# danaesavi/SocialMedia-TextImage-Classification-AuxLosses

Measured on AMD Instinct MI355X. Metric: posts/sec (fwd+bwd) Bernice+ViT-B/16 attn-fusion, bs=64, higher is better.
Workload: dtype bf16; 1 GPU; BASELINE config 2: Bernice+ViT-B/16, attention fusion, no aux loss, bs=64/GPU; step=full train step: fwd + loss + bwd + grad exchange + AdamW + weight refresh, posts_per_gpu=64, image=224, vocab=250002, parallelism=dp1, weights=random-init at true shapes

## Files before the change

socialmedia-textimage-classification-auxlosses_amd/csrc/engine.hip:

```cpp
#include <string>
#include <vector>
#include <cstdlib>
#include <cstdio>
#include "mmhip_common.h"
#include "mmhip_host.h"

using namespace mmhip;

namespace {

struct LayerOff {
    size_t qkv_w, qkv_b, ao_w, ao_b, ln1_w, ln1_b, fc1_w, fc1_b, fc2_w, fc2_b, ln2_w, ln2_b, begin, end;
};
struct LayerW16 {
    size_t qkv, ao, fc1, fc2, qkvT, aoT, fc1T, fc2T;
};
struct TextAct {
    size_t qkv, ctx, pre1, a1, u, h, pre2, out, mean1, rstd1, mean2, rstd2, lse;
    size_t a1p, outp;
};

}

struct mmhip_engine {
// ... 12 lines not shown
    size_t x3_ws[3] = {0, 0, 0}, x3_bytes[3] = {0, 0, 0};
    size_t patch_w16;
    std::vector<TextAct> tact;
    size_t ids_all, mask_all, pos_ids, maskbias, x0, xhat_emb, rstd_emb, x0p = 0;
    bool px = false;
    int bwd_np = 3;
    size_t v_patches, v_pe, v_x, v_ln, v_qkv, v_ctx, v_h, v_out;
    size_t g_partial, g_partial_side, g_det_rows = 0;
    size_t g_lnp[2][2];
    uint8_t* word_row_state = nullptr;
    unsigned* bad_index = nullptr;
    unsigned* guard = nullptr;
    size_t g_set[2][6];
    size_t g_dx, g_dx2, g_dpre, g_ddrop, g_dpre1, g_ddrop1, g_dqkv, g_dctx, g_du;
    size_t h_vpool, h_tpool, h_txt_e, h_img_e, h_txt_n, h_img_n, h_txt_inv, h_img_inv, h_logits;
    size_t h_q, h_qk, h_prob, h_xbar, h_z, h_feats, h_featd, h_out_cls, h_out_tim;
    size_t splitk_ws = 0, splitk_ws_vit = 0; bool has_splitk = false;
    size_t h_d_out_cls, h_d_logits, h_d_out_tim, h_dfeats, h_dpre, h_dz, h_dxcls, h_dxbar, h_dqk, h_dq, h_dtxt_e, h_dimg_e,
        h_dtpool, h_dprepool, h_loss;
    int B = 0, T = 0, Bt = 0; bool itm = false, train_mode = false, fwd_done = false, bwd_begun = false;
    bool skip_itc = false, itc_done = false;
    uint64_t seed = 0;
    size_t ws_base = 0;
    int itc_max_world = 0, itc_world = 1, itc_rank = 0;
    size_t h_g_txt = 0, h_g_img = 0, h_g_rowlse = 0, h_g_collse = 0, h_g_loss = 0, h_g_dtn = 0, h_g_din = 0, h_g_ws = 0;
    bool bd_itc_global = false; float bd_w_itc = 0.f;
    const float *bd_out_cls = nullptr, *bd_logits = nullptr, *bd_out_tim = nullptr, *bd_feats = nullptr;
    hipStream_t side = nullptr;
    int vision_ready_B = 0;
    bool vit_is_long = false;
    hipStream_t side_vit[2] = {nullptr, nullptr};
    hipEvent_t ev_fork = nullptr, ev_vit = nullptr, ev_ready[2] = {nullptr, nullptr}, ev_tn[2] = {nullptr, nullptr};
    hipEvent_t ev_layer[2] = {nullptr, nullptr}, ev_opt = nullptr;
    bool tn_pending[2] = {false, false};
    int cls_only = -1;
    bool cls_compact = false;
    int overlap = -1;
    int part[2] = {-1, -1}, cur_part[2] = {0, 0}; bool part_auto = false;
    int part_bwd = -1;
    int spans_on = 0; hipEvent_t span_ev[6] = {nullptr, nullptr, nullptr, nullptr, nullptr, nullptr}; bool span_set[6] = {false, false, false, false, false, false};
    int span(int i, hipStream_t s) {
        if (!spans_on) return 0;
        if (!span_ev[i]) { hipError_t r = hipEventCreate(&span_ev[i]); if (r != hipSuccess) return (int)r; }
        hipError_t r = hipEventRecord(span_ev[i], s);
        span_set[i] = r == hipSuccess;
        return (int)r;
    }
    int timing = 0;
    struct Ev { hipEvent_t a, b; double flops; int M, N, K, flags, tile, cus; };
    std::vector<Ev> evs; size_t ev_used = 0;

    template <typename U> U* wsp(size_t off) const { return reinterpret_cast<U*>(ws + off); }
    int dt() const { return cfg.dtype; }
    bool clip() const { return cfg.img_kind == MMHIP_IMG_CLIP; }
    int Hv() const { return cfg.hidden_img > 0 ? cfg.hidden_img : cfg.hidden; }
    int Iv() const { return cfg.inter_img > 0 ? cfg.inter_img : cfg.inter; }
    int heads_v() const { return cfg.heads_img > 0 ? cfg.heads_img : cfg.heads; }
    int P() const { return (cfg.image / cfg.patch) * (cfg.image / cfg.patch) + 1; }
    int Kp() const { return 3 * cfg.patch * cfg.patch; }
    int Kpp() const { return (Kp() + 63) / 64 * 64; }
    size_t v_pre_ln_w = 0, v_pre_ln_b = 0;
    float gscale() const { return cfg.loss_scale > 0.f ? cfg.loss_scale : (cfg.dtype == MMHIP_F16 ? 1024.f : 1.f); }
    size_t esz() const { return cfg.dtype == MMHIP_BF16X3 ? 4 : 2; }
};

namespace {

void add_text_layer(ParamTable& b, const mmhip_config& c, int l, LayerOff& o) {
    const int H = c.hidden, I = c.inter;
    const std::string p = "dual_encoder.text_model.encoder.layer." + std::to_string(l) + ".";
    const int g = MMHIP_G_ALWAYS;
    o.begin = b.off[1];
    o.qkv_w = b.add(p + "attention.self.query.weight", 1, g, {H, H});
// ... 245 lines not shown
int run_gemm_pair(mmhip_engine& e, G& g0, G& g1, hipStream_t s) {
    const bool pairable = (e.dt() == DT_BF16 || e.dt() == DT_F16 || (e.dt() == DT_F32 && g0.a.a_pair && g1.a.a_pair)) && g0.a.N == g1.a.N && g0.a.K == g1.a.K;
    mmhip_engine::Ev* ev = nullptr;
    if (e.timing && pairable) {
        if (e.ev_used == e.evs.size()) {
            mmhip_engine::Ev n;
            CHECK_HIP(hipEventCreate(&n.a));
            CHECK_HIP(hipEventCreate(&n.b));
            e.evs.push_back(n);
        }
        ev = &e.evs[e.ev_used];
        CHECK_HIP(hipEventRecord(ev->a, s));
    }
    if (pairable && launch_gemm_nt8_pair(g0.a, g1.a, e.dt(), 0, s)) {
        CHECK_HIP(hipGetLastError());
        if (ev) {
            ev->flops = 2.0 * ((double)g0.a.M + g1.a.M) * (double)g0.a.N * g0.a.K;
            ev->M = g0.a.M + g1.a.M; ev->N = g0.a.N; ev->K = g0.a.K; ev->flags = g0.a.flags | g1.a.flags; ev->tile = -2; ev->cus = 0;
            CHECK_HIP(hipEventRecord(ev->b, s));
            e.ev_used++;
        }
        return 0;
    }
    CHECK_RC(run_gemm(e, g0, s));
    return run_gemm(e, g1, s);
}

int side_init(mmhip_engine& e) {
    if (e.overlap < 0) { const char* v = getenv("MMHIP_OVERLAP"); e.overlap = v ? atoi(v) : 1; }
    if (!e.overlap || e.side) return 0;
    CHECK_HIP(pool_stream(POOL_SIDE, &e.side));
    CHECK_HIP(pool_stream(POOL_VIT, &e.side_vit[0]));
    CHECK_HIP(pool_stream(POOL_VIT_HI, &e.side_vit[1]));
    hipEvent_t* evs[9] = {&e.ev_fork, &e.ev_vit, &e.ev_ready[0], &e.ev_ready[1], &e.ev_tn[0], &e.ev_tn[1], &e.ev_layer[0], &e.ev_layer[1], &e.ev_opt};
    for (auto ev : evs) CHECK_HIP(hipEventCreateWithFlags(ev, hipEventDisableTiming));
    return 0;
}
inline bool use_side(const mmhip_engine& e) { return e.overlap > 0 && e.side && e.timing != 2; }

int refresh_layer(mmhip_engine& e, const float* base, const LayerOff& o, const LayerW16& w, bool transposed, hipStream_t s, int H, int I) {
    CastMat m[4] = {{base + o.qkv_w, e.ws + w.qkv, transposed ? e.ws + w.qkvT : nullptr, 3 * H, H, 0},
                    {base + o.ao_w, e.ws + w.ao, transposed ? e.ws + w.aoT : nullptr, H, H, 0},
                    {base + o.fc1_w, e.ws + w.fc1, transposed ? e.ws + w.fc1T : nullptr, I, H, 0},
                    {base + o.fc2_w, e.ws + w.fc2, transposed ? e.ws + w.fc2T : nullptr, H, I, 0}};
    CHECK_HIP(launch_cast_group(m, 4, e.px ? DT_PAIR : e.dt(), s));
    return 0;
}

int vit_forward(mmhip_engine& e, const float* pixels, hipStream_t s) {
    const mmhip_config& c = e.cfg;
    const int H = e.Hv(), I = e.Iv(), B = e.B, P = e.P(), Kpp = e.Kpp(), dt = e.dt();
    const int Mv = B * P;
    const bool clip = e.clip();
    const float* F = e.frozen;
    const bool px = e.px;
    CHECK_HIP(launch_patchify(pixels, e.ws + e.v_patches, B, c.image, c.patch, Kpp, px ? DT_PAIR : dt, s));
    {
        G g(e.ws + e.v_patches, Kpp, e.ws + e.patch_w16, Kpp, e.ws + e.v_pe, H, B * (P - 1), H, Kpp);
        if (!clip) g.bias(F + e.v_patch_b);
        g.px_in(px);
        part_gemm(e, g, 1);
        CHECK_RC(run_gemm(e, g, s));
    }
    CHECK_HIP(launch_vit_assemble(e.ws + e.v_pe, F + e.v_cls, F + e.v_pos, e.ws + e.v_x, B, P, H, dt, s));
    char* x = e.ws + e.v_x;
    if (clip) {
        LNArgs ln{x, x, F + e.v_pre_ln_w, F + e.v_pre_ln_b, nullptr, nullptr, Mv, H, H, H, c.ln_eps_img};
// ... 259 lines not shown
        CHECK_HIP(launch_fusion_attn_fwd(fa, dt, s));
        CHECK_HIP(launch_small_nt(small(e.wsp<float>(e.h_xbar), H, W + e.fv_w, H, W + e.fv_b, z + H, ZW, Bt, H, H), DT_F32, s));
    } else {
        CHECK_HIP(launch_gather_rows_f32(e.ws + e.v_out, (size_t)P * Hv, z + H, ZW, B, Hv, dt, s));
        if (Bt > B) CHECK_HIP(launch_gather_rows_f32(e.ws + e.v_out, (size_t)P * Hv, z + (size_t)B * ZW + H, ZW, B, Hv, dt, s));
    }
    float* feats = e.wsp<float>(e.h_feats);
    CHECK_HIP(launch_small_nt(small(z, ZW, W + e.fus_w, ZW, W + e.fus_b, feats, H, Bt, H, ZW, ACT_RELU), DT_F32, s));
    CHECK_HIP(launch_elementwise(EW_DROPOUT, feats, nullptr, e.wsp<float>(e.h_featd), (size_t)B * H, 0.f,
                                 make_drop(c.p_head, e.seed, STREAM_HEAD, e.train_mode), s));
    CHECK_HIP(launch_small_nt(small(e.wsp<float>(e.h_featd), H, W + e.cls_w, H, W + e.cls_b, e.wsp<float>(e.h_out_cls), C, B, C, H), DT_F32, s));
    if (e.itm) CHECK_HIP(launch_small_nt(small(feats + (size_t)B * H, H, W + e.tim_w, H, W + e.tim_b, e.wsp<float>(e.h_out_tim), 2, B, 2, H), DT_F32, s));
    if (out_cls) CHECK_HIP(hipMemcpyAsync(out_cls, e.ws + e.h_out_cls, (size_t)B * C * 4, hipMemcpyDeviceToDevice, s));
    if (logits && e.itc_done) CHECK_HIP(hipMemcpyAsync(logits, e.ws + e.h_logits, (size_t)B * B * 4, hipMemcpyDeviceToDevice, s));
    if (out_tim && e.itm) CHECK_HIP(hipMemcpyAsync(out_tim, e.ws + e.h_out_tim, (size_t)B * 2 * 4, hipMemcpyDeviceToDevice, s));
    if (feats_out) CHECK_HIP(hipMemcpyAsync(feats_out, feats, (size_t)B * H * 4, hipMemcpyDeviceToDevice, s));
    return 0;
}

int heads_backward(mmhip_engine& e, hipStream_t s) {
    const mmhip_config& c = e.cfg;
    const int H = c.hidden, E = c.proj_dim, C = c.num_labels, T = e.T, B = e.B, Bt = e.Bt, dt = e.dt();
    const int P = e.P(), Hv = e.Hv(), ZW = H + Hv;
    const float* W = e.train;
    float* Gd = e.grad;
    const float* d_out_cls = e.bd_out_cls ? e.bd_out_cls : e.wsp<float>(e.h_d_out_cls);
    const float* d_logits = e.bd_logits;
    const float* d_out_tim = e.bd_out_tim;
    float* dfeats = e.wsp<float>(e.h_dfeats);
    float* feats = e.wsp<float>(e.h_feats);
    float* z = e.wsp<float>(e.h_z);
    float* dxcls = e.wsp<float>(e.h_dxcls);
    const DropCfg nodrop = make_drop(0.f, 0, 0, false);
    CHECK_HIP(launch_small_nn(small(d_out_cls, C, W + e.cls_w, H, nullptr, dfeats, H, B, H, C), s));
    CHECK_HIP(launch_elementwise(EW_DROPOUT, dfeats, nullptr, dfeats, (size_t)B * H, 0.f, make_drop(c.p_head, e.seed, STREAM_HEAD, e.train_mode), s));
    if (e.bd_feats) CHECK_HIP(launch_elementwise(EW_ADD, dfeats, e.bd_feats, dfeats, (size_t)B * H, 1.f, nodrop, s));
    CHECK_HIP(launch_small_tn(small(d_out_cls, C, e.wsp<float>(e.h_featd), H, nullptr, Gd + e.cls_w, H, B, H, 0, 0, 1), DT_F32, C, s));
    CHECK_HIP(launch_bias_grad_f32(d_out_cls, B, C, C, Gd + e.cls_b, 1, s));
    if (e.itm) {
        if (d_out_tim) {
            CHECK_HIP(launch_small_nn(small(d_out_tim, 2, W + e.tim_w, H, nullptr, dfeats + (size_t)B * H, H, B, H, 2), s));
            CHECK_HIP(launch_small_tn(small(d_out_tim, 2, feats + (size_t)B * H, H, nullptr, Gd + e.tim_w, H, B, H, 0, 0, 1), DT_F32, 2, s));
            CHECK_HIP(launch_bias_grad_f32(d_out_tim, B, 2, 2, Gd + e.tim_b, 1, s));
        } else {
            CHECK_HIP(hipMemsetAsync(dfeats + (size_t)B * H, 0, (size_t)B * H * 4, s));
        }
    }
    float* dpre = e.wsp<float>(e.h_dpre);
    CHECK_HIP(launch_elementwise(EW_RELU_BWD, dfeats, feats, dpre, (size_t)Bt * H, 0.f, nodrop, s));
    CHECK_HIP(launch_small_tn(small(dpre, H, z, ZW, nullptr, Gd + e.fus_w, ZW, Bt, ZW, 0, 0, 1), DT_F32, H, s));
    CHECK_HIP(launch_bias_grad_f32(dpre, Bt, H, H, Gd + e.fus_b, 1, s));
    float* dz = e.wsp<float>(e.h_dz);
    CHECK_HIP(launch_small_nn(small(dpre, H, W + e.fus_w, ZW, nullptr, dz, ZW, Bt, ZW, H), s));
    CHECK_HIP(hipMemcpy2DAsync(dxcls, (size_t)H * 4, dz, (size_t)ZW * 4, (size_t)H * 4, Bt, hipMemcpyDeviceToDevice, s));
    if (c.fusion == MMHIP_FUSION_ATTENTION) {
        const float* dctx = dz + H;
        float* q = e.wsp<float>(e.h_q);
        CHECK_HIP(launch_small_tn(small(dctx, ZW, e.wsp<float>(e.h_xbar), H, nullptr, Gd + e.fv_w, H, Bt, H, 0, 0, 1), DT_F32, H, s));
        CHECK_HIP(launch_bias_grad_f32(dctx, Bt, H, ZW, Gd + e.fv_b, 1, s));
        CHECK_HIP(launch_small_nn(small(dctx, ZW, W + e.fv_w, H, nullptr, e.wsp<float>(e.h_dxbar), H, Bt, H, H), s));
        FusionAttnBwdArgs fb{e.wsp<float>(e.h_dxbar), e.wsp<float>(e.h_prob), e.ws + e.v_out, e.wsp<float>(e.h_dqk), Bt, B, P, H, 1.0f / sqrtf((float)H)};
        CHECK_HIP(launch_fusion_attn_bwd(fb, dt, s));
        CHECK_HIP(launch_small_tn(small(q, H, e.wsp<float>(e.h_dqk), H, nullptr, Gd + e.fk_w, H, Bt, H, 0, 0, 1), DT_F32, H, s));
        CHECK_HIP(launch_small_nt(small(e.wsp<float>(e.h_dqk), H, W + e.fk_w, H, nullptr, e.wsp<float>(e.h_dq), H, Bt, H, H), DT_F32, s));
        CHECK_HIP(launch_small_tn(small(e.wsp<float>(e.h_dq), H, z, ZW, nullptr, Gd + e.fq_w, H, Bt, H, 0, 0, 1), DT_F32, H, s));
        CHECK_HIP(launch_bias_grad_f32(e.wsp<float>(e.h_dq), Bt, H, H, Gd + e.fq_b, 1, s));
        CHECK_HIP(launch_small_nn(small(e.wsp<float>(e.h_dq), H, W + e.fq_w, H, nullptr, dxcls, H, Bt, H, H, ACT_NONE, 1), s));
    }
    if (d_logits || e.bd_itc_global) {
        if (e.bd_itc_global) {
            const int G = e.itc_world * B;
            ItcGlobalBwdArgs gb{};
            gb.txt_n = e.wsp<float>(e.h_g_txt); gb.img_n = e.wsp<float>(e.h_g_img); gb.logit_scale = W + e.logit_scale;
            gb.rowlse = e.wsp<float>(e.h_g_rowlse); gb.collse = e.wsp<float>(e.h_g_collse);
            gb.txt_inv = e.wsp<float>(e.h_txt_inv); gb.img_inv = e.wsp<float>(e.h_img_inv);
            gb.d_txt_n = e.wsp<float>(e.h_g_dtn); gb.d_img_n = e.wsp<float>(e.h_g_din);
            gb.dtxt_e = e.wsp<float>(e.h_dtxt_e); gb.dimg_e = e.wsp<float>(e.h_dimg_e); gb.dlogit_scale = Gd + e.logit_scale;
            gb.ws = e.wsp<float>(e.h_g_ws); gb.G = G; gb.E = E; gb.Bl = B; gb.r0 = e.itc_rank * B;
            gb.scale = e.bd_w_itc * (float)e.itc_world / (2.f * (float)G);
            CHECK_HIP(launch_itc_global_bwd(gb, s));
        } else {
            ItcBwdArgs ib{d_logits, e.wsp<float>(e.h_logits), e.wsp<float>(e.h_txt_n), e.wsp<float>(e.h_img_n), e.wsp<float>(e.h_txt_inv),
                          e.wsp<float>(e.h_img_inv), W + e.logit_scale, e.wsp<float>(e.h_dtxt_e), e.wsp<float>(e.h_dimg_e), Gd + e.logit_scale, B, E};
            CHECK_HIP(launch_itc_bwd(ib, s));
        }
        CHECK_HIP(launch_small_tn(small(e.wsp<float>(e.h_dtxt_e), E, e.wsp<float>(e.h_tpool), H, nullptr, Gd + e.tproj_w, H, B, H, 0, 0, 1), DT_F32, E, s));
        CHECK_HIP(launch_small_tn(small(e.wsp<float>(e.h_dimg_e), E, e.wsp<float>(e.h_vpool), Hv, nullptr, Gd + e.vproj_w, Hv, B, Hv, 0, 0, 1), DT_F32, E, s));
        CHECK_HIP(launch_small_nn(small(e.wsp<float>(e.h_dtxt_e), E, W + e.tproj_w, H, nullptr, e.wsp<float>(e.h_dtpool), H, B, H, E), s));
        CHECK_HIP(launch_elementwise(EW_TANH_BWD, e.wsp<float>(e.h_dtpool), e.wsp<float>(e.h_tpool), e.wsp<float>(e.h_dprepool), (size_t)B * H, 0.f, nodrop, s));
        CHECK_HIP(launch_small_tn(small(e.wsp<float>(e.h_dprepool), H, z, ZW, nullptr, Gd + e.t_pool_w, H, B, H, 0, 0, 1), DT_F32, H, s));
        CHECK_HIP(launch_bias_grad_f32(e.wsp<float>(e.h_dprepool), B, H, H, Gd + e.t_pool_b, 1, s));
        CHECK_HIP(launch_small_nn(small(e.wsp<float>(e.h_dprepool), H, W + e.t_pool_w, H, nullptr, dxcls, H, B, H, H, ACT_NONE, 1), s));
    }
    CHECK_HIP(launch_scatter_cls_rows(dxcls, e.ws + e.g_dx, Bt, e.cls_compact ? 1 : T, H, dt, s, e.gscale()));
    return 0;
}

int text_layer_backward(mmhip_engine& e, int l, hipStream_t s) {
    const mmhip_config& c = e.cfg;
    const int H = c.hidden, I = c.inter, T = e.T, Bt = e.Bt, Mt = Bt * T, dt = e.dt();
    const float* W = e.train;
    float* Gd = e.grad;
    const LayerOff& o = e.txt[l];
    const LayerW16& w = e.txt_w16[l];
    const TextAct& a = e.tact[l];
    const bool px = e.px;
    const int np = e.bwd_np;
    const bool hi1 = px && np == 1;
    const char* x_in = px ? (l ? e.ws + e.tact[l - 1].outp : e.ws + e.x0p) : (l ? e.ws + e.tact[l - 1].out : e.ws + e.x0);
    const bool tr = e.train_mode;
    const int set = l & 1;
    const bool side = use_side(e);
    const bool compact = e.cls_compact && l == c.layers_txt - 1;
    const int Mr = compact ? Bt : Mt, rs = compact ? T * H : H, rmul = compact ? T : 1;
    char *dx = e.ws + e.g_dx, *dx2 = e.ws + e.g_dx2, *dctx = e.ws + e.g_dctx;
    char *dpre2 = e.ws + e.g_set[set][0], *ddrop2 = e.ws + e.g_set[set][1], *du = e.ws + e.g_set[set][2];
    char *dpre1 = e.ws + e.g_set[set][3], *ddrop1 = e.ws + e.g_set[set][4], *dqkv = e.ws + e.g_set[set][5];
    if (side && e.tn_pending[set]) {
        CHECK_HIP(hipStreamWaitEvent(s, e.ev_tn[set], 0));
        e.tn_pending[set] = false;
    }
    const DropCfg d_ffn = make_drop(c.p_hidden, e.seed, stream_ffn_out(l), tr);
    LNBwdArgs b2{dx, e.ws + a.pre2, W + o.ln2_w, e.wsp<float>(a.mean2), e.wsp<float>(a.rstd2), dpre2, nullptr, Gd + o.ln2_w, Gd + o.ln2_b, Mr, H,
                 e.wsp<float>(e.g_lnp[set][0]), 1.0f / e.gscale(), d_ffn.thresh16 ? ddrop2 : nullptr, nullptr, d_ffn, rmul, 1};
    ln_bwd_pair(b2, px, ddrop2, hi1);
    CHECK_HIP(launch_layernorm_bwd(b2, dt, s));
    const char* df = (px || d_ffn.thresh16) ? ddrop2 : dpre2;
    if (e.part_bwd < 0) { const char* v = getenv("MMHIP_PART_BWD"); e.part_bwd = v ? atoi(v) : 0; }
    static int bwd_mask = -1;
    if (bwd_mask < 0) { const char* v = getenv("MMHIP_PART_BWD_MASK"); bwd_mask = v ? atoi(v) : 15; }
    auto part_bwd = [&](G& g, int bit) {
        if (e.part_bwd > 0 && (bwd_mask & bit) && side && g.a.M >= 2048 && g.a.N % 256 == 0 && g.a.K % 64 == 0 && (dt == DT_BF16 || dt == DT_F16)) g.tile(15).grid(e.part_bwd);
    };
    { G g(df, H, e.ws + w.fc2T, H, du, I, Mr, I, H); g.mul_gelu_grad(e.ws + a.u, I).px_in(px, np).px_out(px, hi1); part_bwd(g, 1); CHECK_RC(run_gemm(e, g, s)); }
    static int bt12 = -1;
    if (bt12 < 0) { const char* v = getenv("MMHIP_BWD_TILE12"); bt12 = v ? atoi(v) : 1; }
    const int nt = (bt12 && Mr >= 4096 && Mr <= 8192 && H % 96 == 0) ? 12 : 0;
    { G g(du, I, e.ws + w.fc1T, I, dx2, H, Mr, H, I); g.residual(dpre2, H).px_in(px, np); g.tile(nt); part_bwd(g, 2); CHECK_RC(run_gemm(e, g, s)); }
    const DropCfg d_ao = make_drop(c.p_hidden, e.seed, stream_attn_out(l), tr);
    LNBwdArgs b1{dx2, e.ws + a.pre1, W + o.ln1_w, e.wsp<float>(a.mean1), e.wsp<float>(a.rstd1), dpre1, nullptr, Gd + o.ln1_w, Gd + o.ln1_b, Mr, H,
                 e.wsp<float>(e.g_lnp[set][1]), 1.0f / e.gscale(), d_ao.thresh16 ? ddrop1 : nullptr, nullptr, d_ao, rmul, 1};
    ln_bwd_pair(b1, px, ddrop1, hi1);
    CHECK_HIP(launch_layernorm_bwd(b1, dt, s));
    const char* dout = (px || d_ao.thresh16) ? ddrop1 : dpre1;
    if (compact) {
        { G g(dout, H, e.ws + w.aoT, H, dx2, H, Mr, H, H); g.px_in(px, np).px_out(px, hi1); CHECK_RC(run_gemm(e, g, s)); }
        CHECK_HIP(hipMemsetAsync(dctx, 0, (size_t)Mt * H * e.esz(), s));
        CHECK_HIP(launch_scatter_rows16(dx2, dctx, Bt, (size_t)T * H, H, 0, dt, s));
        CHECK_HIP(hipMemsetAsync(dqkv, 0, (size_t)Mt * 3 * H * e.esz(), s));
    } else {
        G g(dout, H, e.ws + w.aoT, H, dctx, H, Mt, H, H);
        g.px_in(px, np).px_out(px, hi1);
        g.tile((bt12 & 2) ? nt : 0);
        part_bwd(g, 4);
        CHECK_RC(run_gemm(e, g, s));
    }
    AttnBwdArgs ab = attn_bwd_args(e.ws + a.qkv, e.wsp<float>(e.maskbias), e.ws + a.ctx, dctx, e.wsp<float>(a.lse), dqkv, Bt, T, c.heads, H,
                                   make_drop(c.p_attn, e.seed, stream_attn(l), tr));
    attn_pair(ab, px, np);
    ab.q_tiles = compact ? 1 : 0;
    CHECK_HIP(launch_attn_bwd(ab, dt, s));
    hipStream_t ps = s;
    if (side) {
        CHECK_HIP(hipEventRecord(e.ev_ready[set], s));
        CHECK_HIP(hipStreamWaitEvent(e.side, e.ev_ready[set], 0));
        ps = e.side;
    }
    if (compact) {
        { G g(dqkv, 3 * H, e.ws + w.qkvT, 3 * H, dx, H, Mt, H, 3 * H); g.px_in(px, np); CHECK_RC(run_gemm(e, g, s)); }
        CHECK_HIP(launch_scatter_rows16(dpre1, dx, Bt, (size_t)T * H, H, 1, dt, s));
    } else {
        G g(dqkv, 3 * H, e.ws + w.qkvT, 3 * H, dx, H, Mt, H, 3 * H);
        g.residual(dpre1, H).px_in(px, np);
        g.tile(nt);
        part_bwd(g, 8);
        CHECK_RC(run_gemm(e, g, s));
    }
    GemmTNProblem pr[4];
    CHECK_HIP(launch_layernorm_bwd_reduce(b2, ps));
    CHECK_HIP(launch_layernorm_bwd_reduce(b1, ps));
    pr[0] = GemmTNProblem{df, e.ws + a.h, Gd + o.fc2_w, Mr, H, I, H, I, I, 0, Gd + o.fc2_b};
    pr[1] = GemmTNProblem{du, e.ws + a.a1, Gd + o.fc1_w, Mr, I, H, I, H, H, 0, Gd + o.fc1_b};
    pr[2] = GemmTNProblem{dqkv, x_in, Gd + o.qkv_w, Mt, 3 * H, H, 3 * H, H, H, 0, Gd + o.qkv_b};
    pr[3] = GemmTNProblem{dout, e.ws + a.ctx, Gd + o.ao_w, Mr, H, H, H, rs, H, 0, Gd + o.ao_b};
    if (px) {
        pr[1].B = e.ws + a.a1p;
        for (auto& q : pr) tn_pair(q, np);
    }
    {
        const int i = e.side && ps == e.side ? 1 : 0;
        CHECK_HIP(launch_gemm_tn(pr, 4, 0, dt, 0, ps, 1.0f / e.gscale(), e.x3_bytes[i] ? e.ws + e.x3_ws[i] : nullptr, e.x3_bytes[i]));
    }
    if (side) {
        CHECK_HIP(hipEventRecord(e.ev_tn[set], e.side));
        e.tn_pending[set] = true;
    }
    return 0;
}

int backward_finish(mmhip_engine& e, hipStream_t s) {
    for (int set = 0; set < 2; ++set)
        if (e.tn_pending[set]) {
            CHECK_HIP(hipStreamWaitEvent(s, e.ev_tn[set], 0));
            e.tn_pending[set] = false;
        }
    return 0;
}

static unsigned* g_nonfinite = nullptr;
static unsigned* g_skip = nullptr;
inline unsigned* guard_counter(const mmhip_engine& e) { return e.guard ? e.guard : g_nonfinite; }
inline unsigned* guard_flag(const mmhip_engine& e) { return e.guard ? e.guard + 1 : g_skip; }

int embed_backward(mmhip_engine& e, hipStream_t s) {
    const mmhip_config& c = e.cfg;
    const float* W = e.train;
    float* Gd = e.grad;
    EmbedBwdArgs b{};
    b.dx = e.ws + e.g_dx; b.xhat = e.ws + e.xhat_emb; b.rstd = e.wsp<float>(e.rstd_emb); b.gamma = W + e.t_eln_w;
    b.ids = e.wsp<int64_t>(e.ids_all); b.pos_ids = e.wsp<int>(e.pos_ids);
    b.dword = Gd + e.t_word; b.dpos = Gd + e.t_pos; b.dtype = Gd + e.t_type; b.dgamma = Gd + e.t_eln_w; b.dbeta = Gd + e.t_eln_b;
    b.posts = e.Bt; b.T = e.T; b.H = c.hidden; b.pad_id = c.pad_id;
    b.pos_pad_id = c.txt_kind == MMHIP_TXT_XLMR ? c.pad_id : -1;
    b.drop = make_drop(c.p_hidden, e.seed, STREAM_EMBED, e.train_mode);
    b.partial = e.wsp<float>(e.g_partial);
    b.alpha = 1.0f / e.gscale();
    b.row_state = e.word_row_state;
    if (deterministic()) { b.det_rows = e.wsp<float>(e.g_det_rows); b.max_pos = c.max_pos; }
    b.status = guard_flag(e) ? guard_counter(e) : nullptr;
    CHECK_HIP(launch_embed_bwd(b, e.dt(), s));
    return 0;
}

// ... 4 lines not shown
const char* mmhip_version(void) { return "mmhip 0.1 (gfx950)"; }

int mmhip_create(const mmhip_config* cfg, mmhip_handle* out) {
    if (!cfg || !out) return MMHIP_E_INVALID;
    const mmhip_config& c = *cfg;
    if (c.hidden <= 0 || c.hidden % 64 || c.hidden > 1024 || c.heads * 64 != c.hidden || c.inter % 128 || c.hidden % 128) return MMHIP_E_INVALID;
    {
        const int hv = c.hidden_img > 0 ? c.hidden_img : c.hidden, iv = c.inter_img > 0 ? c.inter_img : c.inter, nh = c.heads_img > 0 ? c.heads_img : c.heads;
        if (c.img_kind != MMHIP_IMG_VIT && c.img_kind != MMHIP_IMG_CLIP) return MMHIP_E_INVALID;
        if (hv % 128 || hv > 1024 || nh * 64 != hv || iv % 128 || c.patch < 2 || c.image % c.patch) return MMHIP_E_INVALID;
        if (c.fusion == MMHIP_FUSION_ATTENTION && hv != c.hidden) return MMHIP_E_INVALID;
        const int P = (c.image / c.patch) * (c.image / c.patch) + 1;
        if (P > 608) return MMHIP_E_INVALID;
    }
    if (c.max_text_len > 128 || c.max_text_len < 1 || c.max_posts < 1 || c.max_posts > 1024) return MMHIP_E_INVALID;
    if (c.dtype != MMHIP_BF16 && c.dtype != MMHIP_F16 && c.dtype != MMHIP_BF16X3) return MMHIP_E_INVALID;
    if (c.num_labels < 1 || c.num_labels > 64 || c.proj_dim < 1 || c.proj_dim > 1024) return MMHIP_E_INVALID;
    if (c.txt_kind == MMHIP_TXT_XLMR && c.max_pos < c.max_text_len + c.pad_id + 1) return MMHIP_E_INVALID;
    if (c.txt_kind == MMHIP_TXT_BERT && c.max_pos < c.max_text_len) return MMHIP_E_INVALID;
    mmhip_engine* e = new (std::nothrow) mmhip_engine();
    if (!e) return MMHIP_E_INVALID;
    e->cfg = c;
    if (c.dtype == MMHIP_BF16X3) { const char* v = getenv("MMHIP_X3_PAIRS"); e->px = v ? atoi(v) != 0 : true; }
    if (c.dtype == MMHIP_BF16X3) { const char* v = getenv("MMHIP_X3_BWD"); const int n = v ? atoi(v) : 3; e->bwd_np = n >= 1 && n <= 3 ? n : 3; }
    build_layout(*e);
    build_workspace(*e);
    *out = e;
    return 0;
}
void mmhip_destroy(mmhip_handle h) {
    if (!h) return;
    if (h->side) {
        (void)hipStreamSynchronize(h->side);
        for (hipEvent_t ev : {h->ev_fork, h->ev_vit, h->ev_ready[0], h->ev_ready[1], h->ev_tn[0], h->ev_tn[1], h->ev_layer[0], h->ev_layer[1], h->ev_opt})
            if (ev) (void)hipEventDestroy(ev);
        for (auto sv : h->side_vit) if (sv) (void)hipStreamSynchronize(sv);
        for (auto ev : h->span_ev) if (ev) (void)hipEventDestroy(ev);
    }
    for (auto& ev : h->evs) { (void)hipEventDestroy(ev.a); (void)hipEventDestroy(ev.b); }
    delete h;
}
int mmhip_param_count(mmhip_handle h) { return h ? (int)h->params.size() : MMHIP_E_INVALID; }
int mmhip_param_info_at(mmhip_handle h, int i, mmhip_param_info* out) {
    if (!h || !out || i < 0 || i >= (int)h->params.size()) return MMHIP_E_INVALID;
    *out = h->params[i];
    return 0;
}
uint64_t mmhip_buffer_numel(mmhip_handle h, int buffer) { return !h ? 0 : (buffer == 0 ? h->n_frozen : h->n_train); }
uint64_t mmhip_workspace_bytes(mmhip_handle h) { return h ? h->ws_need : 0; }
int mmhip_reserve_itc_global(mmhip_handle h, int max_world) {
    if (!h || max_world < 0) return MMHIP_E_INVALID;
    if (h->ws) return MMHIP_E_STATE;
    mmhip_engine& e = *h;
    const size_t Bm = e.cfg.max_posts, E = e.cfg.proj_dim, Gm = (size_t)max_world * Bm;
    if (max_world > 1 && Gm > (size_t)ITC_GLOBAL_MAX_G) return MMHIP_E_INVALID;
    e.itc_max_world = max_world > 1 ? max_world : 0;
    e.itc_world = 1; e.itc_rank = 0;
    e.ws_need = e.ws_base;
    if (!e.itc_max_world) return 0;
    Carver w;
    w.off = e.ws_base;
    e.h_g_txt = w.take(Gm * E * 4); e.h_g_img = w.take(Gm * E * 4); e.h_g_rowlse = w.take(Gm * 4); e.h_g_collse = w.take(Gm * 4); e.h_g_loss = w.take(16);
    e.h_g_dtn = w.take(Bm * E * 4); e.h_g_din = w.take(Bm * E * 4); e.h_g_ws = w.take(itc_global_ws_floats((int)Gm, (int)Bm) * 4);
    e.ws_need = w.off;
    return 0;
}
int mmhip_set_itc_global(mmhip_handle h, int world, int rank) {
// ... 173 lines not shown
    a.n_correct = n_correct;
    a.B = e.B; a.C = e.cfg.num_labels;
    CHECK_HIP(launch_loss(a, s));
    if (loss) CHECK_HIP(hipMemcpyAsync(loss, a.loss, 16, hipMemcpyDeviceToDevice, s));
    e.bd_out_cls = a.d_out_cls; e.bd_logits = a.d_logits; e.bd_out_tim = a.d_out_tim; e.bd_feats = nullptr;
    e.bd_itc_global = glob; e.bd_w_itc = w_itc;
    return 0;
}

int mmhip_num_backward_stages(mmhip_handle h) { return h ? h->cfg.layers_txt + 2 : MMHIP_E_INVALID; }

int mmhip_stage_grad_range(mmhip_handle h, int stage, uint64_t* begin, uint64_t* end) {
    if (!h || !begin || !end || stage < 0 || stage > h->cfg.layers_txt + 1) return MMHIP_E_INVALID;
    const mmhip_engine& e = *h;
    if (stage == 0) { *begin = e.heads_begin; *end = e.heads_end; }
    else if (stage <= e.cfg.layers_txt) { const LayerOff& o = e.txt[e.cfg.layers_txt - stage]; *begin = o.begin; *end = o.end; }
    else { *begin = e.emb_begin; *end = e.emb_end; }
    return 0;
}

int mmhip_backward_begin(mmhip_handle h, const float* d_out_cls, const float* d_logits, const float* d_out_tim, const float* d_feats, void* stream) {
    if (!h || !h->fwd_done || !h->grad) return MMHIP_E_STATE;
    mmhip_engine& e = *h;
    if (unsigned* f = guard_flag(e)) CHECK_HIP(hipMemsetAsync(f, 0, 4, (hipStream_t)stream));
    if (d_out_cls || d_logits || d_out_tim || d_feats) {
        if (!d_out_cls) return MMHIP_E_INVALID;
        e.bd_out_cls = d_out_cls; e.bd_logits = d_logits; e.bd_out_tim = d_out_tim; e.bd_feats = d_feats;
        e.bd_itc_global = false;
    } else if (!e.bd_out_cls) {
        return MMHIP_E_STATE;
    }
    e.bwd_begun = true;
    e.tn_pending[0] = e.tn_pending[1] = false;
    return side_init(e);
}
int mmhip_backward_stage(mmhip_handle h, int stage, void* stream) {
    if (!h || !h->bwd_begun) return MMHIP_E_STATE;
    mmhip_engine& e = *h;
    hipStream_t s = (hipStream_t)stream;
    const int L = e.cfg.layers_txt;
    if (stage == 0) return heads_backward(e, s);
    if (stage >= 1 && stage <= L) return text_layer_backward(e, L - stage, s);
    if (stage == L + 1) return embed_backward(e, s);
    return MMHIP_E_INVALID;
}
int mmhip_backward_join_stage(mmhip_handle h, int stage, void* stream) {
    if (!h || !h->bwd_begun) return MMHIP_E_STATE;
    mmhip_engine& e = *h;
    const int L = e.cfg.layers_txt;
    if (stage < 1 || stage > L) return 0;
    const int set = (L - stage) & 1;
    if (e.tn_pending[set]) {
        CHECK_HIP(hipStreamWaitEvent((hipStream_t)stream, e.ev_tn[set], 0));
        e.tn_pending[set] = false;
    }
    return 0;
}
int mmhip_backward_finish(mmhip_handle h, void* stream) {
    if (!h || !h->bwd_begun) return MMHIP_E_STATE;
    return backward_finish(*h, (hipStream_t)stream);
}
int mmhip_backward(mmhip_handle h, const float* d_out_cls, const float* d_logits, const float* d_out_tim, const float* d_feats, void* stream) {
    CHECK_RC(mmhip_backward_begin(h, d_out_cls, d_logits, d_out_tim, d_feats, stream));
    const int n = mmhip_num_backward_stages(h);
    for (int st = 0; st < n; ++st)
        CHECK_RC(mmhip_backward_stage(h, st, stream));
    return mmhip_backward_finish(h, stream);
}

int mmhip_set_nonfinite_counter(uint32_t* device_counter) {
    if ((uintptr_t)device_counter & 3) return MMHIP_E_INVALID;
    g_nonfinite = device_counter;
    g_skip = nullptr;
    return 0;
}
int mmhip_set_step_guard(uint32_t* device_words2) {
    if ((uintptr_t)device_words2 & 3) return MMHIP_E_INVALID;
    g_nonfinite = device_words2;
    g_skip = device_words2 ? device_words2 + 1 : nullptr;
    return 0;
}
int mmhip_set_guard(mmhip_handle h, uint32_t* device_words2) {
// ... 188 lines not shown
    for (int l = 0; l < L; ++l)
        if (!layer_done[l]) CHECK_RC(refresh_layer(e, e.train, e.txt[l], e.txt_w16[l], true, s, e.cfg.hidden, e.cfg.inter));
    if (rows_due) {
        if (cb) CHECK_RC(cb(user, MMHIP_CB_FINISH_ROWS));
        if (!e.word_row_state) return MMHIP_E_STATE;
        CHECK_RC(adamw_rows_impl(e.train + w0, e.grad + w0, adam_m + w0, adam_v + w0, (int)V, (int)H, e.word_row_state, lr, beta1, beta2, eps,
                                    weight_decay, step, grad_scale, 1, stream, gc, gf));
    }
    return e.span(5, s);
}

int mmhip_train_step(mmhip_handle h, const int64_t* ids, const int64_t* mask, const float* pixels, const int64_t* tim_ids,
                     const int64_t* tim_mask, const int64_t* lbl_tim, const int64_t* onehot, const float* class_w, int B, int T,
                     uint64_t seed, int use_itc, int use_itm, float w_cls, float w_itc, float w_itm, float* adam_m, float* adam_v,
                     float lr, float beta1, float beta2, float eps, float weight_decay, int step, float grad_scale, float* loss,
                     int* n_correct, void* stream) {
    return train_step_impl(h, ids, mask, pixels, tim_ids, tim_mask, lbl_tim, onehot, class_w, B, T, seed, use_itc, use_itm, w_cls, w_itc, w_itm,
                           adam_m, adam_v, lr, beta1, beta2, eps, weight_decay, step, grad_scale, loss, n_correct, stream, nullptr, nullptr);
}
int mmhip_train_step_dp(mmhip_handle h, const int64_t* ids, const int64_t* mask, const float* pixels, const int64_t* tim_ids,
                        const int64_t* tim_mask, const int64_t* lbl_tim, const int64_t* onehot, const float* class_w, int B, int T,
                        uint64_t seed, int use_itc, int use_itm, float w_cls, float w_itc, float w_itm, float* adam_m, float* adam_v,
                        float lr, float beta1, float beta2, float eps, float weight_decay, int step, float grad_scale, float* loss,
                        int* n_correct, void* stream, mmhip_exchange_cb on_stage, void* user) {
    if (!on_stage) return MMHIP_E_INVALID;
    return train_step_impl(h, ids, mask, pixels, tim_ids, tim_mask, lbl_tim, onehot, class_w, B, T, seed, use_itc, use_itm, w_cls, w_itc, w_itm,
                           adam_m, adam_v, lr, beta1, beta2, eps, weight_decay, step, grad_scale, loss, n_correct, stream, on_stage, user);
}

int mmhip_step_spans(mmhip_handle h, int enable, float* ms) {
    if (!h) return MMHIP_E_INVALID;
    mmhip_engine& e = *h;
    if (ms) {
        for (int i = 0; i < 5; ++i) ms[i] = -1.f;
        if (e.span_set[0]) {
            for (int i = 1; i < 6; ++i) {
                if (!e.span_set[i]) continue;
                CHECK_HIP(hipEventSynchronize(e.span_ev[i]));
                float t = 0.f;
                if (hipEventElapsedTime(&t, e.span_ev[0], e.span_ev[i]) == hipSuccess) ms[i - 1] = t;
            }
        }
    }
    e.spans_on = enable;
    if (!enable) for (int i = 0; i < 6; ++i) e.span_set[i] = false;
    return 0;
}
int mmhip_gemm_timing(mmhip_handle h, int enable, int reset, double* ms, uint64_t* launches, double* flops) {
    if (!h) return MMHIP_E_INVALID;
    mmhip_engine& e = *h;
    if (ms || launches || flops) {
        double tms = 0, tf = 0;
        for (size_t i = 0; i < e.ev_used; ++i) {
            CHECK_HIP(hipEventSynchronize(e.evs[i].b));
            float t = 0;
            CHECK_HIP(hipEventElapsedTime(&t, e.evs[i].a, e.evs[i].b));
            tms += t; tf += e.evs[i].flops;
        }
        if (ms) *ms = tms;
        if (launches) *launches = e.ev_used;
        if (flops) *flops = tf;
    }
    if (reset) e.ev_used = 0;
    e.timing = enable < 0 ? 0 : (enable > 2 ? 2 : enable);
    return 0;
}

int mmhip_gemm_timing_by_shape(mmhip_handle h, char* out, uint64_t capacity) {
    if (!h || !out || capacity < 2) return MMHIP_E_INVALID;
    mmhip_engine& e = *h;
    struct Row { int M, N, K, flags, tile, cus; int n; double ms, flops; };
    std::vector<Row> rows;
    for (size_t i = 0; i < e.ev_used; ++i) {
        const auto& ev = e.evs[i];
        CHECK_HIP(hipEventSynchronize(ev.b));
        float t = 0;
        CHECK_HIP(hipEventElapsedTime(&t, ev.a, ev.b));
        Row* r = nullptr;
// ... 22 lines not shown
```

Baseline: 6355 posts/s.

## Offload head weight-gradient GEMMs to side stream and trim CLS-only text backward

Moves the weight and bias gradient reductions of the classifier, fusion, attention-fusion and pooler heads onto the side stream, gated by an event, so they run concurrently with the data-gradient chain on the main stream. A join is added before stage 1 and in backward_finish. Separately, in the compact (CLS-only) last text layer, a lean path for non-f32 dtypes writes the attention-output backward GEMM straight into dctx and zeroes dqkv with a 2D memset, replacing the scatter path, and flags attention backward with Sq_live=1. More profiling span events are also added, at the cost of extra stream and event bookkeeping.

```diff
diff --git a/socialmedia-textimage-classification-auxlosses_amd/csrc/engine.hip b/socialmedia-textimage-classification-auxlosses_amd/csrc/engine.hip
--- a/socialmedia-textimage-classification-auxlosses_amd/csrc/engine.hip
+++ b/socialmedia-textimage-classification-auxlosses_amd/csrc/engine.hip
@@ -68,13 +68,15 @@
     hipStream_t side_vit[2] = {nullptr, nullptr};
     hipEvent_t ev_fork = nullptr, ev_vit = nullptr, ev_ready[2] = {nullptr, nullptr}, ev_tn[2] = {nullptr, nullptr};
     hipEvent_t ev_layer[2] = {nullptr, nullptr}, ev_opt = nullptr;
-    bool tn_pending[2] = {false, false};
+    hipEvent_t ev_heads_in = nullptr, ev_heads = nullptr;
+    bool tn_pending[2] = {false, false}, heads_pending = false;
     int cls_only = -1;
     bool cls_compact = false;
     int overlap = -1;
     int part[2] = {-1, -1}, cur_part[2] = {0, 0}; bool part_auto = false;
     int part_bwd = -1;
-    int spans_on = 0; hipEvent_t span_ev[6] = {nullptr, nullptr, nullptr, nullptr, nullptr, nullptr}; bool span_set[6] = {false, false, false, false, false, false};
+    static constexpr int N_SPAN = 8;
+    int spans_on = 0; hipEvent_t span_ev[N_SPAN] = {}; bool span_set[N_SPAN] = {};
     int span(int i, hipStream_t s) {
         if (!spans_on) return 0;
         if (!span_ev[i]) { hipError_t r = hipEventCreate(&span_ev[i]); if (r != hipSuccess) return (int)r; }
@@ -386,7 +388,8 @@
     CHECK_HIP(pool_stream(POOL_SIDE, &e.side));
     CHECK_HIP(pool_stream(POOL_VIT, &e.side_vit[0]));
     CHECK_HIP(pool_stream(POOL_VIT_HI, &e.side_vit[1]));
-    hipEvent_t* evs[9] = {&e.ev_fork, &e.ev_vit, &e.ev_ready[0], &e.ev_ready[1], &e.ev_tn[0], &e.ev_tn[1], &e.ev_layer[0], &e.ev_layer[1], &e.ev_opt};
+    hipEvent_t* evs[11] = {&e.ev_fork, &e.ev_vit, &e.ev_ready[0], &e.ev_ready[1], &e.ev_tn[0], &e.ev_tn[1], &e.ev_layer[0], &e.ev_layer[1], &e.ev_opt,
+                           &e.ev_heads_in, &e.ev_heads};
     for (auto ev : evs) CHECK_HIP(hipEventCreateWithFlags(ev, hipEventDisableTiming));
     return 0;
 }
@@ -712,40 +715,50 @@
     float* z = e.wsp<float>(e.h_z);
     float* dxcls = e.wsp<float>(e.h_dxcls);
     const DropCfg nodrop = make_drop(0.f, 0, 0, false);
+    const bool off = use_side(e);
+    hipStream_t ps = off ? e.side : s;
+    auto inputs_ready = [&]() -> int {
+        if (off) {
+            CHECK_HIP(hipEventRecord(e.ev_heads_in, s));
+            CHECK_HIP(hipStreamWaitEvent(e.side, e.ev_heads_in, 0));
+        }
+        return 0;
+    };
     CHECK_HIP(launch_small_nn(small(d_out_cls, C, W + e.cls_w, H, nullptr, dfeats, H, B, H, C), s));
     CHECK_HIP(launch_elementwise(EW_DROPOUT, dfeats, nullptr, dfeats, (size_t)B * H, 0.f, make_drop(c.p_head, e.seed, STREAM_HEAD, e.train_mode), s));
     if (e.bd_feats) CHECK_HIP(launch_elementwise(EW_ADD, dfeats, e.bd_feats, dfeats, (size_t)B * H, 1.f, nodrop, s));
-    CHECK_HIP(launch_small_tn(small(d_out_cls, C, e.wsp<float>(e.h_featd), H, nullptr, Gd + e.cls_w, H, B, H, 0, 0, 1), DT_F32, C, s));
-    CHECK_HIP(launch_bias_grad_f32(d_out_cls, B, C, C, Gd + e.cls_b, 1, s));
     if (e.itm) {
-        if (d_out_tim) {
-            CHECK_HIP(launch_small_nn(small(d_out_tim, 2, W + e.tim_w, H, nullptr, dfeats + (size_t)B * H, H, B, H, 2), s));
-            CHECK_HIP(launch_small_tn(small(d_out_tim, 2, feats + (size_t)B * H, H, nullptr, Gd + e.tim_w, H, B, H, 0, 0, 1), DT_F32, 2, s));
-            CHECK_HIP(launch_bias_grad_f32(d_out_tim, B, 2, 2, Gd + e.tim_b, 1, s));
-        } else {
-            CHECK_HIP(hipMemsetAsync(dfeats + (size_t)B * H, 0, (size_t)B * H * 4, s));
-        }
+        if (d_out_tim) CHECK_HIP(launch_small_nn(small(d_out_tim, 2, W + e.tim_w, H, nullptr, dfeats + (size_t)B * H, H, B, H, 2), s));
+        else CHECK_HIP(hipMemsetAsync(dfeats + (size_t)B * H, 0, (size_t)B * H * 4, s));
     }
     float* dpre = e.wsp<float>(e.h_dpre);
     CHECK_HIP(launch_elementwise(EW_RELU_BWD, dfeats, feats, dpre, (size_t)Bt * H, 0.f, nodrop, s));
-    CHECK_HIP(launch_small_tn(small(dpre, H, z, ZW, nullptr, Gd + e.fus_w, ZW, Bt, ZW, 0, 0, 1), DT_F32, H, s));
-    CHECK_HIP(launch_bias_grad_f32(dpre, Bt, H, H, Gd + e.fus_b, 1, s));
     float* dz = e.wsp<float>(e.h_dz);
     CHECK_HIP(launch_small_nn(small(dpre, H, W + e.fus_w, ZW, nullptr, dz, ZW, Bt, ZW, H), s));
+    CHECK_RC(inputs_ready());
+    CHECK_HIP(launch_small_tn(small(d_out_cls, C, e.wsp<float>(e.h_featd), H, nullptr, Gd + e.cls_w, H, B, H, 0, 0, 1), DT_F32, C, ps));
+    CHECK_HIP(launch_bias_grad_f32(d_out_cls, B, C, C, Gd + e.cls_b, 1, ps));
+    if (e.itm && d_out_tim) {
+        CHECK_HIP(launch_small_tn(small(d_out_tim, 2, feats + (size_t)B * H, H, nullptr, Gd + e.tim_w, H, B, H, 0, 0, 1), DT_F32, 2, ps));
+        CHECK_HIP(launch_bias_grad_f32(d_out_tim, B, 2, 2, Gd + e.tim_b, 1, ps));
+    }
+    CHECK_HIP(launch_small_tn(small(dpre, H, z, ZW, nullptr, Gd + e.fus_w, ZW, Bt, ZW, 0, 0, 1), DT_F32, H, ps));
+    CHECK_HIP(launch_bias_grad_f32(dpre, Bt, H, H, Gd + e.fus_b, 1, ps));
     CHECK_HIP(hipMemcpy2DAsync(dxcls, (size_t)H * 4, dz, (size_t)ZW * 4, (size_t)H * 4, Bt, hipMemcpyDeviceToDevice, s));
     if (c.fusion == MMHIP_FUSION_ATTENTION) {
         const float* dctx = dz + H;
         float* q = e.wsp<float>(e.h_q);
-        CHECK_HIP(launch_small_tn(small(dctx, ZW, e.wsp<float>(e.h_xbar), H, nullptr, Gd + e.fv_w, H, Bt, H, 0, 0, 1), DT_F32, H, s));
-        CHECK_HIP(launch_bias_grad_f32(dctx, Bt, H, ZW, Gd + e.fv_b, 1, s));
         CHECK_HIP(launch_small_nn(small(dctx, ZW, W + e.fv_w, H, nullptr, e.wsp<float>(e.h_dxbar), H, Bt, H, H), s));
         FusionAttnBwdArgs fb{e.wsp<float>(e.h_dxbar), e.wsp<float>(e.h_prob), e.ws + e.v_out, e.wsp<float>(e.h_dqk), Bt, B, P, H, 1.0f / sqrtf((float)H)};
         CHECK_HIP(launch_fusion_attn_bwd(fb, dt, s));
-        CHECK_HIP(launch_small_tn(small(q, H, e.wsp<float>(e.h_dqk), H, nullptr, Gd + e.fk_w, H, Bt, H, 0, 0, 1), DT_F32, H, s));
         CHECK_HIP(launch_small_nt(small(e.wsp<float>(e.h_dqk), H, W + e.fk_w, H, nullptr, e.wsp<float>(e.h_dq), H, Bt, H, H), DT_F32, s));
-        CHECK_HIP(launch_small_tn(small(e.wsp<float>(e.h_dq), H, z, ZW, nullptr, Gd + e.fq_w, H, Bt, H, 0, 0, 1), DT_F32, H, s));
-        CHECK_HIP(launch_bias_grad_f32(e.wsp<float>(e.h_dq), Bt, H, H, Gd + e.fq_b, 1, s));
         CHECK_HIP(launch_small_nn(small(e.wsp<float>(e.h_dq), H, W + e.fq_w, H, nullptr, dxcls, H, Bt, H, H, ACT_NONE, 1), s));
+        CHECK_RC(inputs_ready());
+        CHECK_HIP(launch_small_tn(small(dctx, ZW, e.wsp<float>(e.h_xbar), H, nullptr, Gd + e.fv_w, H, Bt, H, 0, 0, 1), DT_F32, H, ps));
+        CHECK_HIP(launch_bias_grad_f32(dctx, Bt, H, ZW, Gd + e.fv_b, 1, ps));
+        CHECK_HIP(launch_small_tn(small(q, H, e.wsp<float>(e.h_dqk), H, nullptr, Gd + e.fk_w, H, Bt, H, 0, 0, 1), DT_F32, H, ps));
+        CHECK_HIP(launch_small_tn(small(e.wsp<float>(e.h_dq), H, z, ZW, nullptr, Gd + e.fq_w, H, Bt, H, 0, 0, 1), DT_F32, H, ps));
+        CHECK_HIP(launch_bias_grad_f32(e.wsp<float>(e.h_dq), Bt, H, H, Gd + e.fq_b, 1, ps));
     }
     if (d_logits || e.bd_itc_global) {
         if (e.bd_itc_global) {
@@ -764,16 +777,21 @@
                           e.wsp<float>(e.h_img_inv), W + e.logit_scale, e.wsp<float>(e.h_dtxt_e), e.wsp<float>(e.h_dimg_e), Gd + e.logit_scale, B, E};
             CHECK_HIP(launch_itc_bwd(ib, s));
         }
-        CHECK_HIP(launch_small_tn(small(e.wsp<float>(e.h_dtxt_e), E, e.wsp<float>(e.h_tpool), H, nullptr, Gd + e.tproj_w, H, B, H, 0, 0, 1), DT_F32, E, s));
-        CHECK_HIP(launch_small_tn(small(e.wsp<float>(e.h_dimg_e), E, e.wsp<float>(e.h_vpool), Hv, nullptr, Gd + e.vproj_w, Hv, B, Hv, 0, 0, 1), DT_F32, E, s));
         CHECK_HIP(launch_small_nn(small(e.wsp<float>(e.h_dtxt_e), E, W + e.tproj_w, H, nullptr, e.wsp<float>(e.h_dtpool), H, B, H, E), s));
         CHECK_HIP(launch_elementwise(EW_TANH_BWD, e.wsp<float>(e.h_dtpool), e.wsp<float>(e.h_tpool), e.wsp<float>(e.h_dprepool), (size_t)B * H, 0.f, nodrop, s));
-        CHECK_HIP(launch_small_tn(small(e.wsp<float>(e.h_dprepool), H, z, ZW, nullptr, Gd + e.t_pool_w, H, B, H, 0, 0, 1), DT_F32, H, s));
-        CHECK_HIP(launch_bias_grad_f32(e.wsp<float>(e.h_dprepool), B, H, H, Gd + e.t_pool_b, 1, s));
         CHECK_HIP(launch_small_nn(small(e.wsp<float>(e.h_dprepool), H, W + e.t_pool_w, H, nullptr, dxcls, H, B, H, H, ACT_NONE, 1), s));
+        CHECK_RC(inputs_ready());
+        CHECK_HIP(launch_small_tn(small(e.wsp<float>(e.h_dtxt_e), E, e.wsp<float>(e.h_tpool), H, nullptr, Gd + e.tproj_w, H, B, H, 0, 0, 1), DT_F32, E, ps));
+        CHECK_HIP(launch_small_tn(small(e.wsp<float>(e.h_dimg_e), E, e.wsp<float>(e.h_vpool), Hv, nullptr, Gd + e.vproj_w, Hv, B, Hv, 0, 0, 1), DT_F32, E, ps));
+        CHECK_HIP(launch_small_tn(small(e.wsp<float>(e.h_dprepool), H, z, ZW, nullptr, Gd + e.t_pool_w, H, B, H, 0, 0, 1), DT_F32, H, ps));
+        CHECK_HIP(launch_bias_grad_f32(e.wsp<float>(e.h_dprepool), B, H, H, Gd + e.t_pool_b, 1, ps));
+    }
+    if (off) {
+        CHECK_HIP(hipEventRecord(e.ev_heads, e.side));
+        e.heads_pending = true;
     }
     CHECK_HIP(launch_scatter_cls_rows(dxcls, e.ws + e.g_dx, Bt, e.cls_compact ? 1 : T, H, dt, s, e.gscale()));
-    return 0;
+    return e.span(6, s);
 }
 
 int text_layer_backward(mmhip_engine& e, int l, hipStream_t s) {
@@ -823,7 +841,11 @@
     ln_bwd_pair(b1, px, ddrop1, hi1);
     CHECK_HIP(launch_layernorm_bwd(b1, dt, s));
     const char* dout = (px || d_ao.thresh16) ? ddrop1 : dpre1;
-    if (compact) {
+    const bool lean = compact && dt != DT_F32;
+    if (lean) {
+        { G g(dout, H, e.ws + w.aoT, H, dctx, rs, Mr, H, H); CHECK_RC(run_gemm(e, g, s)); }
+        CHECK_HIP(hipMemset2DAsync(dqkv, (size_t)3 * H * e.esz(), 0, (size_t)H * e.esz(), (size_t)Mt, s));
+    } else if (compact) {
         { G g(dout, H, e.ws + w.aoT, H, dx2, H, Mr, H, H); g.px_in(px, np).px_out(px, hi1); CHECK_RC(run_gemm(e, g, s)); }
         CHECK_HIP(hipMemsetAsync(dctx, 0, (size_t)Mt * H * e.esz(), s));
         CHECK_HIP(launch_scatter_rows16(dx2, dctx, Bt, (size_t)T * H, H, 0, dt, s));
@@ -839,6 +861,7 @@
                                    make_drop(c.p_attn, e.seed, stream_attn(l), tr));
     attn_pair(ab, px, np);
     ab.q_tiles = compact ? 1 : 0;
+    if (lean) ab.Sq_live = 1;
     CHECK_HIP(launch_attn_bwd(ab, dt, s));
     hipStream_t ps = s;
     if (side) {
@@ -875,10 +898,19 @@
         CHECK_HIP(hipEventRecord(e.ev_tn[set], e.side));
         e.tn_pending[set] = true;
     }
-    return 0;
-}
-
+    if (l == c.layers_txt - 1) CHECK_RC(e.span(7, s));
+    return 0;
+}
+
+int join_heads(mmhip_engine& e, hipStream_t s) {
+    if (e.heads_pending) {
+        CHECK_HIP(hipStreamWaitEvent(s, e.ev_heads, 0));
+        e.heads_pending = false;
+    }
+    return 0;
+}
 int backward_finish(mmhip_engine& e, hipStream_t s) {
+    CHECK_RC(join_heads(e, s));
     for (int set = 0; set < 2; ++set)
         if (e.tn_pending[set]) {
             CHECK_HIP(hipStreamWaitEvent(s, e.ev_tn[set], 0));
@@ -949,7 +981,8 @@
     if (!h) return;
     if (h->side) {
         (void)hipStreamSynchronize(h->side);
-        for (hipEvent_t ev : {h->ev_fork, h->ev_vit, h->ev_ready[0], h->ev_ready[1], h->ev_tn[0], h->ev_tn[1], h->ev_layer[0], h->ev_layer[1], h->ev_opt})
+        for (hipEvent_t ev : {h->ev_fork, h->ev_vit, h->ev_ready[0], h->ev_ready[1], h->ev_tn[0], h->ev_tn[1], h->ev_layer[0], h->ev_layer[1], h->ev_opt,
+                              h->ev_heads_in, h->ev_heads})
             if (ev) (void)hipEventDestroy(ev);
         for (auto sv : h->side_vit) if (sv) (void)hipStreamSynchronize(sv);
         for (auto ev : h->span_ev) if (ev) (void)hipEventDestroy(ev);
@@ -1189,6 +1222,7 @@
     }
     e.bwd_begun = true;
     e.tn_pending[0] = e.tn_pending[1] = false;
+    e.heads_pending = false;
     return side_init(e);
 }
 int mmhip_backward_stage(mmhip_handle h, int stage, void* stream) {
@@ -1205,6 +1239,7 @@
     if (!h || !h->bwd_begun) return MMHIP_E_STATE;
     mmhip_engine& e = *h;
     const int L = e.cfg.layers_txt;
+    if (stage == 0) return join_heads(e, (hipStream_t)stream);
     if (stage < 1 || stage > L) return 0;
     const int set = (L - stage) & 1;
     if (e.tn_pending[set]) {
@@ -1459,9 +1494,10 @@
     if (!h) return MMHIP_E_INVALID;
     mmhip_engine& e = *h;
     if (ms) {
-        for (int i = 0; i < 5; ++i) ms[i] = -1.f;
+        const int n = (enable & 2) ? mmhip_engine::N_SPAN : 6;
+        for (int i = 0; i < n - 1; ++i) ms[i] = -1.f;
         if (e.span_set[0]) {
-            for (int i = 1; i < 6; ++i) {
+            for (int i = 1; i < n; ++i) {
                 if (!e.span_set[i]) continue;
                 CHECK_HIP(hipEventSynchronize(e.span_ev[i]));
                 float t = 0.f;
@@ -1470,7 +1506,7 @@
         }
     }
     e.spans_on = enable;
-    if (!enable) for (int i = 0; i < 6; ++i) e.span_set[i] = false;
+    if (!enable) for (int i = 0; i < mmhip_engine::N_SPAN; ++i) e.span_set[i] = false;
     return 0;
 }
 int mmhip_gemm_timing(mmhip_handle h, int enable, int reset, double* ms, uint64_t* launches, double* flops) {
```

Result: no change. 6397 posts/s (median of 6 runs) (+0.7%).
